# xyzy/jubatus

Measured on AMD Instinct MI355X. Metric: train_samples_per_sec, higher is better.
Workload: dtype fp32

## Files before the change

jubatus_amd/csrc/hip/jb_vc_state.hpp:

```cpp
#pragma once
#include <stdint.h>

#include "jb_serial_layout.hpp"

namespace jb {
namespace vc {

enum : int { kNew = 0, kRetry = 1, kDone = 2, kDense = 3 };
enum : int {
  S_MAGIC = 0, S_BEG, S_BEND, S_STATUS, S_LW, S_T, S_NCAND, S_PEND, S_WHY, S_NUPD, S_NSLOTS, S_VIOL,
  S_DONEB, S_NVALID, S_RETRYW, S_WEND,
  S_WINDOWS, S_RETRIES, S_STEPS, S_ROUNDS, S_WASTED, S_REFRESH, S_EXACT, S_CAND, S_UPD, S_SAT, S_TICKS,
  S_NONC, S_PH0, S_PH1, S_PH2, S_PH3, S_PH4, S_PHW, S_WIDE, S_DENSE_PM,
  S_DCHUNK,
  S_STEPPED,
  S_NCHUNK,
  S_BBEG,
  S_CSMODE,
  S_CSN,
  S_NWORDS = 64
};
enum : int { kWhyEnd = 0, kWhySat = 1, kWhyDense = 2 };
constexpr int64_t kDenseChunk0 = 8192, kDenseChunkMax = 1 << 20;

constexpr int kSpSlotBytes = 98304;
__host__ __device__ constexpr int sp_nslot(int lc) {
  return kSpSlotBytes / (8 * lc) > 1024 ? 1024 : kSpSlotBytes / (8 * lc);
}
__device__ __forceinline__ void sp_buckets(int row, int nb, int* b1, int* b2) {
  const uint32_t h1 = (uint32_t)row * 0x9E3779B1u;
  uint32_t h2 = ((uint32_t)row ^ 0x5bd1e995u) * 0x85EBCA77u;
  h2 ^= h2 >> 13;
  h2 *= 0xC2B2AE35u;
  *b1 = (int)__umulhi(h1, (uint32_t)nb);
  int c = (int)__umulhi(h2, (uint32_t)nb);
  if (c == *b1) c = c + 1 == nb ? 0 : c + 1;
  *b2 = c;
}
__device__ __forceinline__ int sp_find(const int32_t* key, int nb, int32_t row) {
  if (row < 0) return -1;
  int b1, b2;
  sp_buckets(row, nb, &b1, &b2);
  const int4 k1 = reinterpret_cast<const int4*>(key)[b1];
  const int4 k2 = reinterpret_cast<const int4*>(key)[b2];
  int s = -1;
  s = k1.x == row ? 4 * b1 : s;
  s = k1.y == row ? 4 * b1 + 1 : s;
  s = k1.z == row ? 4 * b1 + 2 : s;
  s = k1.w == row ? 4 * b1 + 3 : s;
  s = k2.x == row ? 4 * b2 : s;
  s = k2.y == row ? 4 * b2 + 1 : s;
  s = k2.z == row ? 4 * b2 + 2 : s;
  s = k2.w == row ? 4 * b2 + 3 : s;
  return s;
}

__device__ inline int64_t seg_estimate(const int64_t* st) {
  const int64_t wins = st[S_WINDOWS], stepped = st[S_STEPPED];
  const int64_t committed = st[S_BEG] - st[S_BBEG] - stepped;
  int64_t per = committed > 0 && wins > 0 ? committed / wins : 2048;
  per = per < 1024 ? 1024 : per;
  return wins + st[S_RETRIES] + (stepped + per - 1) / per;
}

}
}
```

jubatus_amd/csrc/hip/serial.hip:

```cpp
#include "jb_linear.hpp"
#include "jb_serial_layout.hpp"
#include <cstdio>
#include <cstdlib>
#include <algorithm>
#include <mutex>
#include <unordered_map>

namespace jb {

constexpr int kCommitThreads = 512;
constexpr int kDBits = 14;
constexpr int kDCap = 1 << kDBits;
constexpr int kDProbe = 32;
constexpr int kDFull = kDCap * 5 / 8;
constexpr int kBloomBits = 16;
constexpr int kSerialNF = 16;
constexpr float kSlackGuard = 1e-4f;
constexpr int kStepBits = 8;
constexpr int kStepCap = 1 << kStepBits;
constexpr int kStepList = 64;
constexpr int kSerialSegments = 4;
constexpr int kSerialSegmentsBig = 48;
constexpr int64_t kSerialBigBatch = 16384;
constexpr int kVerifiedSegmentsMin = 8;
constexpr int kVerifiedSegmentsMax = 2048;
constexpr int kRescoreWaste = 16;
constexpr int kScoreMaxBlocks = 8192;
#ifndef JB_SERIAL_TIMING
#define JB_SERIAL_TIMING 0
#endif
constexpr bool kSerialTiming = JB_SERIAL_TIMING != 0;
__device__ __forceinline__ uint64_t stamp() { return kSerialTiming ? clock64() : 0; }

template <int LC>
__device__ __forceinline__ void sample_scores_ro(const int32_t* __restrict__ fidx,
                                                 const float* __restrict__ fval, int64_t beg, int n,
                                                 const float* __restrict__ W, int lane,
                                                 float (&acc)[Lanes<LC>::K]) {
  using L = Lanes<LC>;
  const int g = lane / L::LW;
  const int l0 = lane % L::LW;
#pragma unroll
  for (int k = 0; k < L::K; ++k) acc[k] = 0.f;
  for (int j = g; j < n; j += L::G) {
    const int32_t idx = fidx[beg + j];
    const float x = fval[beg + j];
    if (idx >= 0) {
      const float* wr = W + (int64_t)idx * LC + l0;
#pragma unroll
      for (int k = 0; k < L::K; ++k) acc[k] += x * wr[64 * k];
    }
  }
#pragma unroll
  for (int off = L::LW; off < 64; off <<= 1) {
#pragma unroll
    for (int k = 0; k < L::K; ++k) acc[k] += __shfl_xor(acc[k], off, 64);
  }
}

template <int LC>
__device__ __forceinline__ float margin_of(const float (&acc)[Lanes<LC>::K], int y,
                                           const bool (&act)[Lanes<LC>::K], int lane, int* lstar,
                                           float* sy_out, float* best_out) {
  using L = Lanes<LC>;
  const int l0 = lane % L::LW;
  float sy = 0.f, best = -INFINITY;
  int bl = -1;
#pragma unroll
  for (int k = 0; k < L::K; ++k) {
    const int l = l0 + 64 * k;
    if (l == y) sy = acc[k];
    if (act[k] && l != y && acc[k] > best) { best = acc[k]; bl = l; }
  }
  sy = __shfl(sy, y % L::LW, 64);
  argmax_wrong<L::LW>(best, bl);
  *lstar = bl;
  *sy_out = sy;
  *best_out = bl >= 0 ? best : 0.f;
  return sy - (bl >= 0 ? best : 0.f);
}

__device__ __forceinline__ float decision_slack(int method, float margin, float nrm, bool has_l,
                                                float C, float sy, float best) {
  float s;
  switch (method) {
    case PERCEPTRON: s = margin; break;
    case PA: case PA1: case PA2:
      if (!(nrm > 0.f)) return INFINITY;
      s = margin - 1.f;
      break;
    case CW: {
      if (!(nrm > 0.f)) return INFINITY;
      s = margin - C * (has_l ? 2.f : 1.f) * nrm;
      break;
    }
    default:
      s = margin - 1.f;
      break;
  }
  const float guard = kSlackGuard * (1.f + fabsf(sy) + fabsf(best));
  if (method == PERCEPTRON ? !(s > guard) : !(s >= guard)) return -1.f;
  return s - guard;
}

template <int LC>
__global__ __launch_bounds__(256) void serial_score_kernel(
    const int64_t* __restrict__ row_ptr, const int32_t* __restrict__ fidx,
    const float* __restrict__ fval, const int32_t* __restrict__ labels,
// ... 470 lines not shown
      if (tid == k) {
        if (!loaded) load_features<NF>(fi, fx, live, nf, fb, fidx, fval);
        s_n = nf;
        s_y = yl;
        s_fb = fb;
        if (nf <= NF)
          for (int u = 0; u < nf; ++u) { s_fi[u] = fi[u]; s_fx[u] = fx[u]; }
      }
      if (wv == 0) {
        d.step_clear(lane);
        __builtin_amdgcn_wave_barrier();
        if (lane == 0) s_sn = 0;
      }
      lds_barrier();
      { const uint64_t t = stamp(); ph[2] += t - tc; tc = t; }
      if (wv == 0) {
        asm volatile("s_waitcnt vmcnt(0)" ::: "memory");
        const int n = s_n;
        bool up;
        if (kStaged && n <= NF)
          up = commit_staged<(LC <= 32 ? LC : 32)>(s_fi, s_fx, n, s_y, W, P, act[0], lane, method, C,
                                                   touched, d);
        else
          up = commit_sample<LC>(fidx, fval, s_fb, n, s_y, W, P, act, lane, method, C, touched, d);
        if (up) ++n_upd; else ++n_waste;
        if (lane == 0) s_waste = n_waste;
      }
      lim = k;
      ++steps;
      ++n_steps;
      { const uint64_t t = stamp(); ph[3] += t - tc; tc = t; }
      lds_barrier();
      { const uint64_t t = stamp(); ph[4] += t - tc; tc = t; }
      tw = stamp();
      if (s_sat || steps > bail_after || (rescore_waste > 0 && s_waste > rescore_waste)) {
        stop = p + k + 1;
        why = s_sat ? kStopSaturated : steps > bail_after ? kStopDense : kStopRescore;
        break;
      }
      if (loaded && open && tid > k && sl >= 0.f) {
        if (s_sn > kStepList || nf > NF) {
          bnd = full_bound();
        } else {
          bnd += d.step_bound<NF>(fi, fx);
        }
      }
    }
    ++n_rounds;
    const bool counted = live && !(sl != sl) && j < stop;
    const uint64_t cm = __builtin_amdgcn_ballot_w64(counted);
    if (lane == 0 && cm != 0) atomicAdd(&s_valid, (unsigned)__popcll(cm));
    if (stop != end) break;
  }
  __syncthreads();
  auto put = [&](int i, int64_t v) { tail[i] = seg == 0 ? v : tail[i] + v; };
  if (lane == 0) put(kTailBoundWave0 + wv, (int64_t)wwork);
  if (tid == 0) {
    tail[kTailStart] = stop;
    tail[kTailEnd] = end;
    tail[kTailReason] = why;
    put(kTailSteps, n_steps);
    put(kTailRounds, n_rounds);
    put(kTailSegments, 1);
    for (int i = 0; i < 6; ++i) put(kTailBoundPhase0 + i, (int64_t)ph[i]);
    put(kTailBoundWall, kSerialTiming ? (int64_t)(wall_clock64() - w0) : 0);
    put(kTailBoundCycles,
        (int64_t)(stamp() - tc) + (int64_t)(ph[0] + ph[1] + ph[2] + ph[3] + ph[4] + ph[5]));
    if (stats != nullptr && s_valid > 0) atomicAdd(stats + 1, (unsigned long long)s_valid);
  }
  if (tid == 0 && stats != nullptr && n_upd > 0) atomicAdd(stats, (unsigned long long)n_upd);
}

}

extern "C" int64_t jb_serial_scratch_bytes(int64_t n_max) {
  return jb::VcScratch::bytes(n_max > 0 ? n_max : 1);
}

extern "C" int64_t jb_serial_scratch_bytes_lc(int64_t n_max, int LC) {
  return LC > 64 ? jb::BoundScratch::bytes(n_max > 0 ? n_max : 1) : jb_serial_scratch_bytes(n_max);
}

enum : int { kSeenReason = 0, kSeenSegments, kSeenSegEst, kSeenWords };
static_assert(jb::kTailSegments == jb::kTailReason + 1, "one copy reads back both");
static std::mutex& seen_mu() {
  static std::mutex mu;
  return mu;
}
static std::unordered_map<void*, int64_t*>& seen_map() {
  static std::unordered_map<void*, int64_t*> seen;
  return seen;
}
static int64_t* segments_seen(void* scratch) {
  std::lock_guard<std::mutex> g(seen_mu());
  auto& seen = seen_map();
  auto it = seen.find(scratch);
  if (it != seen.end()) return it->second;
  int64_t* p = nullptr;
  if (hipHostMalloc((void**)&p, kSeenWords * sizeof(int64_t), hipHostMallocDefault) != hipSuccess) return nullptr;
  p[kSeenReason] = jb::kStopDone;
  p[kSeenSegments] = 128;
  p[kSeenSegEst] = 0;
  seen[scratch] = p;
  return p;
}

extern "C" int jb_vcommit_prepare(const int64_t* row_ptr, const int32_t* fidx, const float* fval,
                                  const int32_t* labels, const int64_t* stream_ptr, int nstreams, int64_t n_max,
                                  float* W, float* S, const int32_t* active, int LC, int method, float C,
                                  unsigned long long* stats, uint8_t* touched, void* scratch, int nseg,
                                  hipStream_t stream);

extern "C" int jb_serial_scratch_forget(void* scratch) {
  std::lock_guard<std::mutex> g(seen_mu());
  auto& seen = seen_map();
  auto it = seen.find(scratch);
  if (it == seen.end()) return 0;
  (void)hipHostFree(it->second);
  seen.erase(it);
  return 1;
}

static int segment_budget(int64_t n_max, int64_t prev, int64_t est, int64_t why) {
  if (n_max < jb::kSerialBigBatch) return jb::kVerifiedSegmentsMin;
  if (why != jb::kStopDone && why != jb::kStopDense) return jb::kVerifiedSegmentsMax;
  static const std::pair<int, int> slack = [] {
    const char* e = getenv("JB_VC_SEG_SLACK");
    int d = 2, c = 8;
    if (e != nullptr && sscanf(e, "%d,%d", &d, &c) != 2) { d = 2; c = 8; }
    return std::make_pair(d > 0 ? d : 2, c >= 0 ? c : 8);
  }();
  prev = std::max(prev, est);
  return (int)std::min<int64_t>(jb::kVerifiedSegmentsMax,
                                std::max<int64_t>(jb::kVerifiedSegmentsMin,
                                                  prev + prev / slack.first + slack.second));
}

extern "C" int jb_serial_prepare(const int64_t* row_ptr, const int32_t* fidx, const float* fval,
                                 const int32_t* labels, const int64_t* stream_ptr, int nstreams,
                                 int64_t n_max, float* W, float* S, const int32_t* active, int LC,
                                 int method, float C, unsigned long long* stats, uint8_t* touched,
                                 void* scratch, int64_t scratch_bytes, int bail_after,
                                 hipStream_t stream) {
  if (nstreams <= 0 || n_max <= 0) return 0;
  if (scratch == nullptr || scratch_bytes < jb_serial_scratch_bytes_lc(n_max, LC)) return -3;
  if (method >= jb::CW && S == nullptr) return -4;
  int64_t* tail = (int64_t*)scratch;
  if (LC <= 64) {
    volatile int64_t* seen = segments_seen(scratch);
    const int nseg = seen != nullptr
                         ? segment_budget(n_max, seen[kSeenSegments], seen[kSeenSegEst], seen[kSeenReason])
                         : segment_budget(n_max, 0, 0, jb::kStopDone);
    const int rc = jb_vcommit_prepare(row_ptr, fidx, fval, labels, stream_ptr, nstreams, n_max, W, S, active,
                                      LC, method, C, stats, touched, scratch, nseg, stream);
    if (rc == 0 && seen != nullptr) {
      int64_t* host = const_cast<int64_t*>(seen);
      (void)hipMemcpyAsync(host + kSeenReason, tail + jb::kTailReason, 2 * sizeof(int64_t), hipMemcpyDeviceToHost,
                           stream);
      (void)hipMemcpyAsync(host + kSeenSegEst, tail + jb::kTailSegEst, sizeof(int64_t), hipMemcpyDeviceToHost,
                           stream);
    }
    return rc;
  }
  float* slack = (float*)((uint8_t*)scratch + jb::BoundScratch::slack_offset());
  float* l1n = (float*)((uint8_t*)scratch + jb::BoundScratch::l1_offset(n_max));
  const int64_t blocks = std::min<int64_t>((n_max * 64 + 255) / 256, jb::kScoreMaxBlocks);
  const int nseg = n_max >= jb::kSerialBigBatch ? jb::kSerialSegmentsBig : jb::kSerialSegments;
  static_assert(jb::kTailStart == 0 && jb::kTailEnd == 1, "the tail doubles as a one-stream stream_ptr");
  for (int seg = 0; seg < nseg; ++seg) {
    const int waste = seg + 1 < nseg ? jb::kRescoreWaste : 0;
    const int64_t* sp = seg == 0 ? stream_ptr : tail;
    const int ns = seg == 0 ? nstreams : 1;
    const int64_t* why = seg == 0 ? nullptr : tail + jb::kTailReason;
#define JB_SERIAL(L)                                                                              \
  hipLaunchKernelGGL((jb::serial_score_kernel<L>), dim3((unsigned)blocks), dim3(256), 0, stream,  \
                     row_ptr, fidx, fval, labels, sp, ns, W, active, method, C, slack, l1n, why); \
  hipLaunchKernelGGL((jb::serial_commit_kernel<L>), dim3(1), dim3(jb::kCommitThreads), 0, stream, \
                     row_ptr, fidx, fval, labels, sp, ns, W, S, active, method, C, slack, l1n,    \
                     stats, touched, tail, bail_after, seg, waste);                               \
  break;
    switch (LC) {
      case 128: JB_SERIAL(128)
      case 256: JB_SERIAL(256)
      case 512: JB_SERIAL(512)
      case 1024: JB_SERIAL(1024)
      default: return -1;
    }
#undef JB_SERIAL
  }
  return (int)hipGetLastError();
}
```

jubatus_amd/csrc/hip/vcommit.hip:

```cpp
#include <string.h>

#include <type_traits>

#include "jb_commit.hpp"
#include "jb_vc_state.hpp"

namespace jb {
namespace vc {

using dc::Geo;
constexpr int kFCMax = 2;
constexpr int kRec = 16 * kFCMax;
constexpr int64_t kLwMin = 2048, kLwMax = kVcWindowMax, kLwInit = 8192;
constexpr int kBitWords = kVcBitWords;
constexpr float kTInit = 0.5f, kTMin = 0.125f, kTMax = 64.f;
constexpr int64_t kMagic = 0x56434f4d4d495433LL;
constexpr int kRetryForce = 3;

__device__ __forceinline__ float st_T(const int64_t* st) { return __int_as_float((int)st[S_T]); }
__device__ __forceinline__ int64_t ld_st(const int64_t* p) {
  return __hip_atomic_load(p, __ATOMIC_RELAXED, __HIP_MEMORY_SCOPE_AGENT);
}
__device__ __forceinline__ bool live(int status) { return status == kNew || status == kRetry; }

__device__ __forceinline__ float frcp(float x) { return __builtin_amdgcn_rcpf(x); }
__device__ __forceinline__ bool step_coeffs_fast(int method, float margin, float var, float nrm, bool has_l, float C,
                                                 float* tau, float* beta) {
  switch (method) {
    case PERCEPTRON:
      if (margin <= 0.f) { *tau = 1.f; *beta = 0.f; return true; }
      return false;
    case PA: case PA1: case PA2: {
      const float loss = 1.f - margin;
      if (!(loss > 0.f && nrm > 0.f)) return false;
      const float sq = (has_l ? 2.f : 1.f) * nrm;
      if (method == PA) *tau = loss * frcp(sq);
      else if (method == PA1) *tau = fminf(C, loss * frcp(sq));
      else *tau = loss * frcp(sq + 0.5f * frcp(C));
      *beta = 0.f;
      return true;
    }
    case CW: {
      if (!(var > 0.f)) return false;
      const float phi = C;
      const float b = 1.f + 2.f * phi * margin;
      const float disc = b * b - 8.f * phi * (margin - phi * var);
      const float gamma = (-b + sqrtf(fmaxf(disc, 0.f))) * frcp(4.f * phi * var);
      if (!(gamma > 0.f)) return false;
      *tau = gamma; *beta = 2.f * gamma * phi;
      return true;
    }
    case AROW:
      if (!(margin < 1.f)) return false;
      *beta = frcp(var + frcp(C));
      *tau = (1.f - margin) * *beta;
      return true;
    case NHERD: {
      if (!(margin < 1.f)) return false;
      *tau = (1.f - margin) * frcp(var + frcp(C));
      const float cv = 1.f + C * var;
      *beta = (C * C * var + 2.f * C) * frcp(cv * cv);
      return true;
    }
    default: return false;
  }
}
__device__ __forceinline__ float dprec_fast(int method, float beta, float x, float s) {
  const float bx2 = beta * x * x;
  return method == CW ? bx2 : bx2 * frcp(1.f - bx2 * s);
}

__global__ __launch_bounds__(256) void vc_init_kernel(int64_t* __restrict__ st, const int64_t* __restrict__ sp,
                                                      int nstreams, unsigned long long* __restrict__ bits,
                                                      int64_t* __restrict__ tail, float t_force,
                                                      int32_t* __restrict__ g_key, float* __restrict__ g_rmax,
                                                      int dense_pm) {
  for (int i = threadIdx.x; i < kBitWords; i += blockDim.x) bits[i] = 0ull;
  const bool fresh = st[S_MAGIC] != kMagic;
  if (fresh)
    for (int i = threadIdx.x; i < 1024; i += blockDim.x) { g_key[i] = -1; g_rmax[i] = 0.f; }
  __syncthreads();
  if (threadIdx.x != 0) return;
  if (fresh) {
    for (int i = 0; i < S_NWORDS; ++i) st[i] = 0;
    st[S_MAGIC] = kMagic;
    st[S_LW] = kLwInit;
    st[S_T] = __float_as_int(kTInit);
  }
  if (t_force > 0.f) st[S_T] = __float_as_int(t_force);
  const int64_t beg = sp[0], bend = sp[nstreams];
  st[S_BEG] = beg;
  st[S_BEND] = bend;
  st[S_WEND] = beg;
  st[S_STATUS] = beg < bend ? kNew : kDone;
  for (int i = S_NCAND; i <= S_RETRYW; ++i) st[i] = 0;
  for (int i = S_WINDOWS; i < S_NWORDS; ++i) st[i] = 0;
// ... 139 lines not shown
    const int64_t pn = st[S_NCAND], pu = st[S_NUPD];
    st[S_CSMODE] = (cs_min > 0 && ncand >= cs_min && pu * 1000 >= (int64_t)cs_pm * (pn > 0 ? pn : 1)) ? 1 : 0;
    st[S_NCAND] = ncand;
    st[S_WEND] = we;
  }
  const int64_t nwaves = (int64_t)gridDim.x * (blockDim.x >> 6);
  const int g = lane / L::LW;
  const int l0 = lane % L::LW;
  const bool la = l0 < LC && active[l0] != 0;
  for (int64_t k = ((int64_t)blockIdx.x * blockDim.x + tid) >> 6; k < ncand; k += nwaves) {
    int lo = 0, hi = nw - 1;
    while (lo < hi) {
      const int mid = (lo + hi + 1) >> 1;
      if (s_pref[mid] <= k) lo = mid; else hi = mid - 1;
    }
    unsigned long long word = bits[lo];
    for (int j = (int)k - s_pref[lo]; j > 0; --j) word &= word - 1;
    const int pos = 64 * lo + (__ffsll((long long)word) - 1);
    const int64_t s = beg + pos;
    int n;
    float acc, q;
    wave_score<LC>(row_ptr, fidx, fval, W, s, lane, la, &n, &acc, &q);
    const int64_t fb = row_ptr[s];
    if (lane < kRec) {
      const bool in = lane < n;
      FI[k * kRec + lane] = in ? fidx[fb + lane] : -1;
      FX[k * kRec + lane] = in ? fval[fb + lane] : 0.f;
    }
    if (lane == 0 && n > 16) atomicOr((unsigned long long*)&st[S_WIDE], 1ull);
    if (lane < LC) S0[k * LC + lane] = acc;
    (void)g;
    const int y = labels[s];
    if (y < 0 || y >= LC) {
      if (lane == 0) AUX[k] = make_int4(dc::aux_pack(-1, -1, n), __float_as_int(q), __float_as_int(1.f), pos);
      continue;
    }
    int bl;
    const float sl0 = wave_slack<LC>(acc, y, la, lane, method, C, q, &bl);
    if (lane == 0) AUX[k] = make_int4(dc::aux_pack(y, bl, n), __float_as_int(q), __float_as_int(sl0), pos);
    if (P == nullptr) continue;
    if (lane < kRec) {
      float2 pp = make_float2(1.f, 1.f);
      if (lane < n) {
        const int32_t idx = fidx[fb + lane];
        if (idx >= 0) {
          pp.x = P[(int64_t)idx * LC + y];
          if (bl >= 0) pp.y = P[(int64_t)idx * LC + bl];
        }
      }
      PP0[k * kRec + lane] = pp;
    }
  }
}

template <int LC, int FC>
struct Raw {
  int32_t fi[FC];
  float fx[FC];
  float2 pp[FC];
  float s[Geo<LC>::K];
  int aux;
  float nrm;
  float slack0;
  int pos;
};

template <int LC, int FC>
struct Samp {
  int32_t fi[FC];
  float fx[FC];
  float py[FC];
  float pl[FC];
  float s[Geo<LC>::K];
  int y;
  int ls0;
  int nf;
  float nrm;
  float slack0;
  int pos;
};

struct __attribute__((aligned(16))) Stamp { float sid, dy, dl, rmax; };

template <int LC, int MT, int R_, int PD_, int FC_>
__global__ __launch_bounds__(64) void vc_commit_kernel(
    int64_t* __restrict__ st, const float* __restrict__ W, const float* __restrict__ P,
    const int32_t* __restrict__ active, float C, const float* __restrict__ S0_k,
    const int4* __restrict__ AUX_k, const float2* __restrict__ PP0_k, const int32_t* __restrict__ FI_k,
    const float* __restrict__ FX_k, int32_t* __restrict__ g_key, float* __restrict__ g_rmax,
    float* __restrict__ g_dw, float* __restrict__ g_dp, int prof) {
  using Gm = Geo<LC>;
  using Rw = Raw<LC, FC_>;
  using S = Samp<LC, FC_>;
  constexpr int kFC = FC_;
  constexpr int kNFM = 16 * FC_;
  constexpr int kR = R_;
  constexpr int kNS = 4 * R_;
  constexpr int kPD = PD_;
  constexpr int K = Gm::K;
  constexpr int NSLOT = Gm::NSLOT;
  constexpr int method = MT;
  constexpr bool use_s = MT >= CW;
  constexpr bool use_nrm = MT == PA || MT == PA1 || MT == PA2 || MT == CW;
  constexpr float kG = dc::kGuard;
  if (!live((int)st[S_STATUS])) return;
  if (st[S_CSMODE] == 1) return;
  if ((st[S_WIDE] != 0) != (FC_ == 2)) return;
  __shared__ __attribute__((aligned(16))) float s_dw[NSLOT * LC + Gm::PAD];
  __shared__ __attribute__((aligned(16))) float s_dp[use_s ? NSLOT * LC + Gm::PAD : 4];
  __shared__ __attribute__((aligned(16))) int32_t s_key[NSLOT];
  __shared__ __attribute__((aligned(16))) Stamp s_sg[NSLOT + 1];

  const int lane = threadIdx.x;
  const int sub = lane & 15;
  const int G = lane >> 4;
  const uint64_t t_k0 = __builtin_amdgcn_s_memrealtime();
  const uint64_t t_c0 = __builtin_amdgcn_s_memtime();
  {
    float4* dw4 = reinterpret_cast<float4*>(s_dw);
    float4* dp4 = reinterpret_cast<float4*>(s_dp);
    const float4 z = make_float4(0.f, 0.f, 0.f, 0.f);
    for (int i = lane; i < (NSLOT * LC + Gm::PAD) / 4; i += 64) {
      dw4[i] = z;
      if (use_s) dp4[i] = z;
    }
    for (int i = lane; i < NSLOT; i += 64) s_key[i] = -1;
    for (int i = lane; i <= NSLOT; i += 64) s_sg[i] = Stamp{__int_as_float(-1), 0.f, 0.f, 0.f};
  }
  int act[K];
#pragma unroll
  for (int k = 0; k < K; ++k) {
    const int lab = sub + 16 * k;
    act[k] = (lab < LC && active[lab] != 0) ? 1 : 0;
  }
  const int64_t ncand = (int64_t)dc::in_vgpr((uint64_t)st[S_NCAND]);
  const int64_t wb = (int64_t)dc::in_vgpr((uint64_t)st[S_BEG]);
  const int64_t we = (int64_t)dc::in_vgpr((uint64_t)st[S_WEND]);
  const float* __restrict__ S0 = dc::in_vgpr(S0_k);
  const int4* __restrict__ AUX = dc::in_vgpr(AUX_k);
  const float2* __restrict__ PP0 = dc::in_vgpr(PP0_k);
  const int32_t* __restrict__ FI = dc::in_vgpr(FI_k);
  const float* __restrict__ FX = dc::in_vgpr(FX_k);

  auto load_raw = [&](int64_t k0, Rw (&rw)[kR]) {
#pragma unroll
    for (int r = 0; r < kR; ++r) {
      int64_t j = k0 + G * kR + r;
      j = j < ncand ? j : ncand - 1;
      j = j < 0 ? 0 : j;
#pragma unroll
      for (int c = 0; c < kFC; ++c) {
        const int64_t o = j * kRec + c * 16 + sub;
        rw[r].fi[c] = dc::gld(FI + o);
        rw[r].fx[c] = dc::gld(FX + o);
        if (use_s) rw[r].pp[c] = dc::gld(PP0 + o);
      }
#pragma unroll
      for (int k = 0; k < K; ++k) {
        const int lab = sub + 16 * k;
        rw[r].s[k] = dc::gld(S0 + j * LC + (lab < LC ? lab : LC - 1));
      }
      const int* a = reinterpret_cast<const int*>(AUX + j);
      rw[r].aux = dc::gld(a);
      rw[r].slack0 = __int_as_float(dc::gld(a + 2));
      rw[r].pos = dc::gld(a + 3);
      if (use_nrm) rw[r].nrm = __int_as_float(dc::gld(a + 1));
    }
  };
  auto unpack = [&](int64_t k0, const Rw (&rw)[kR], S (&sm)[kR]) {
#pragma unroll
    for (int r = 0; r < kR; ++r) {
      const bool ok = k0 + G * kR + r < ncand;
#pragma unroll
      for (int c = 0; c < kFC; ++c) {
        sm[r].fi[c] = ok ? rw[r].fi[c] : -1;
        sm[r].fx[c] = ok ? rw[r].fx[c] : 0.f;
        sm[r].py[c] = (use_s && ok) ? rw[r].pp[c].x : 1.f;
        sm[r].pl[c] = (use_s && ok) ? rw[r].pp[c].y : 1.f;
      }
#pragma unroll
      for (int k = 0; k < K; ++k) sm[r].s[k] = (ok && sub + 16 * k < LC) ? rw[r].s[k] : 0.f;
      const int aux = rw[r].aux;
      sm[r].y = ok ? dc::aux_y(aux) : -1;
      sm[r].ls0 = (use_s && ok) ? dc::aux_ls(aux) : -1;
      sm[r].nf = ok ? dc::aux_nf(aux) : 0;
      sm[r].nrm = (use_nrm && ok) ? rw[r].nrm : 0.f;
      sm[r].slack0 = ok ? rw[r].slack0 : 1.f;
      sm[r].pos = rw[r].pos;
    }
  };

  S sc[kR];
  Rw pf[kPD][kR];
#pragma unroll
  for (int i = 0; i < kPD; ++i) load_raw((int64_t)i * kNS, pf[i]);

  int stopped = 0;
  int64_t pend = we;
  int why = kWhyEnd;
  int n_steps = 0, n_exact = 0;
  __shared__ int s_cnt[4];
  __shared__ unsigned long long s_ph[5];
  if (lane < 4) s_cnt[lane] = 0;
  if (lane < 5) s_ph[lane] = 0;
  auto bump = [&](int i) __attribute__((always_inline)) {
    if (lane == 0) s_cnt[i] += 1;
  };
  const uint64_t kLead = 0x0001000100010001ull;

  const bool kProf = prof != 0;

  uint64_t tp = kProf ? __builtin_amdgcn_s_memtime() : 0;
  auto stamp = [&](int i) __attribute__((always_inline)) {
    if (!kProf) return;
    const uint64_t t = __builtin_amdgcn_s_memtime();
    if (lane == 0) s_ph[i] += t - tp;
    tp = t;
  };
  auto round = [&](int64_t k0) __attribute__((always_inline)) {
    int alive[kR], unsafe[kR], exact[kR];
    float slack[kR];
    int slot[kR][kFC];
    bool widew = false;
#pragma unroll
    for (int r = 0; r < kR; ++r) {
      alive[r] = (sc[r].y >= 0 && sc[r].y < LC) ? 1 : 0;
      widew |= alive[r] && sc[r].nf > 16;
    }
    const bool two = kFC == 2 && __builtin_amdgcn_ballot_w64(widew) != 0;
#pragma unroll
    for (int r = 0; r < kR; ++r) {
      const bool ok = alive[r] && sc[r].nf <= kNFM;
      slot[r][0] = ok ? dc::cache_find<LC>(s_key, sc[r].fi[0]) : -1;
      if (kFC == 2) slot[r][kFC - 1] = (two && ok) ? dc::cache_find<LC>(s_key, sc[r].fi[kFC - 1]) : -1;
    }
    auto make_exact = [&](int after) {
      bool need[kR];
      bool anyneed = false;
#pragma unroll
      for (int r = 0; r < kR; ++r) {
        need[r] = alive[r] && !exact[r] && sc[r].nf <= kNFM && G * kR + r > after && !(slack[r] > 0.f);
        anyneed |= need[r];
      }
      if (__builtin_amdgcn_ballot_w64(anyneed) == 0) return;
#pragma unroll
      for (int r = 0; r < kR; ++r) {
        if (__builtin_amdgcn_ballot_w64(need[r]) == 0) continue;
        float t[K];
#pragma unroll
        for (int k = 0; k < K; ++k) t[k] = sc[r].s[k];
        dc::row_correct<LC, kFC>(s_dw, slot[r], sc[r].fx, sub, two, t);
        int ls;
        float sy, best;
        const float m = dc::group_margin<LC>(t, sc[r].y, act, sub, &ls, &sy, &best);
        const float sl = dc::slack_of(method, m, sc[r].nrm, ls >= 0, C, sy, best);
        if (need[r]) {
#pragma unroll
          for (int k = 0; k < K; ++k) sc[r].s[k] = t[k];
          slack[r] = sl;
          exact[r] = 1;
          if (sub == 0) ++n_exact;
        }
      }
    };
#pragma unroll
    for (int r = 0; r < kR; ++r) {
      float bsum = 0.f;
#pragma unroll
      for (int c = 0; c < kFC; ++c)
        bsum += slot[r][c] >= 0 ? fabsf(sc[r].fx[c]) * s_sg[slot[r][c]].rmax : 0.f;
      slack[r] = sc[r].slack0 - 2.f * (1.f + 4.f * kG) * row16_sum(bsum);
      exact[r] = 0;
    }
    make_exact(-1);
    stamp(0);
#pragma unroll
    for (int r = 0; r < kR; ++r) unsafe[r] = (alive[r] && (sc[r].nf > kNFM || !(slack[r] > 0.f))) ? 1 : 0;

    int lim = -1;
    for (;;) {
      int k = dc::kInf;
#pragma unroll
      for (int r = 0; r < kR; ++r) {
        const uint64_t b = __builtin_amdgcn_ballot_w64(unsafe[r] && G * kR + r > lim) & kLead;
        if (b != 0) {
// ... 175 lines not shown
            cy = row16_sum(cy);
            cl = row16_sum(cl);
            if (exact[r]) {
#pragma unroll
              for (int kk = 0; kk < K; ++kk) {
                const int lab = sub + 16 * kk;
                if (lab == yk) sc[r].s[kk] += cy;
                if (lab == lk) sc[r].s[kk] += cl;
              }
            }
            slack[r] -= (fabsf(cy) + fabsf(cl)) * (1.f + 4.f * kG);
            if (exact[r] && !(slack[r] > 0.f)) {
              int ls2;
              float sy2, best2;
              const float m2 = dc::group_margin<LC>(sc[r].s, sc[r].y, act, sub, &ls2, &sy2, &best2);
              slack[r] = dc::slack_of(method, m2, sc[r].nrm, ls2 >= 0, C, sy2, best2);
            }
          }
          make_exact(k);
#pragma unroll
          for (int r = 0; r < kR; ++r)
            if (G * kR + r > k) unsafe[r] = (alive[r] && (sc[r].nf > kNFM || !(slack[r] > 0.f))) ? 1 : 0;
        }
        return 0;
      };
      int stop_code = 0;
      switch (rk) {
        case 0: stop_code = step_of(std::integral_constant<int, 0>{}); break;
        case 1: if constexpr (kR > 1) stop_code = step_of(std::integral_constant<int, (kR > 1 ? 1 : 0)>{}); break;
        case 2: if constexpr (kR > 2) stop_code = step_of(std::integral_constant<int, (kR > 2 ? 2 : 0)>{}); break;
        default: if constexpr (kR > 3) stop_code = step_of(std::integral_constant<int, (kR > 3 ? 3 : 0)>{}); break;
      }
      stamp(4);
      if (stop_code) break;
      lim = k;
    }
    bump(3);
  };
  for (int64_t p0 = 0; p0 < ncand && !stopped; p0 += kPD * kNS) {
#pragma unroll
    for (int u = 0; u < kPD; ++u) {
      const int64_t p = p0 + u * kNS;
      unpack(p, pf[u], sc);
      load_raw(p + kPD * kNS, pf[u]);
      if (p < ncand && !stopped) round(p);
    }
  }
  int nslots = 0;
  for (int i = lane; i < NSLOT; i += 64) {
    const int32_t key = s_key[i];
    g_key[i] = key;
    g_rmax[i] = s_sg[i].rmax;
    nslots += key >= 0;
  }
  {
    constexpr int Q = LC / 4;
    for (int i = lane; i < NSLOT * Q; i += 64) {
      if (s_key[i / Q] < 0) continue;
      reinterpret_cast<float4*>(g_dw)[i] = reinterpret_cast<const float4*>(s_dw)[i];
      if (use_s) reinterpret_cast<float4*>(g_dp)[i] = reinterpret_cast<const float4*>(s_dp)[i];
    }
  }
#pragma unroll
  for (int off = 1; off < 64; off <<= 1) nslots += __shfl_xor(nslots, off, 64);
  if (lane == 0) {
    st[S_PEND] = pend;
    st[S_WHY] = why;
    st[S_NUPD] = s_cnt[0];
    st[S_NSLOTS] = nslots;
    st[S_STEPS] += n_steps;
    st[S_ROUNDS] += s_cnt[3];
    st[S_WASTED] += s_cnt[1];
    st[S_REFRESH] += s_cnt[2];
    st[S_EXACT] += n_exact;
    st[S_CAND] += ncand;
    st[S_TICKS] += (int64_t)(__builtin_amdgcn_s_memrealtime() - t_k0);
    if (kProf) {
      for (int i = 0; i < 5; ++i) st[S_PH0 + i] += (int64_t)s_ph[i];
      st[S_PHW] += (int64_t)(__builtin_amdgcn_s_memtime() - t_c0);
    }
  }
}

template <int LC>
__global__ __launch_bounds__(256) void vc_verify_kernel(
    int64_t* __restrict__ st, const int64_t* __restrict__ row_ptr, const int32_t* __restrict__ fidx,
    const float* __restrict__ fval, const int32_t* __restrict__ labels, const float* __restrict__ SL,
    unsigned long long* __restrict__ bits, const int32_t* __restrict__ g_key,
    const float* __restrict__ g_rmax, const float* __restrict__ g_dw, const float* __restrict__ g_dp,
    float* __restrict__ W, float* __restrict__ P, uint8_t* __restrict__ touched,
    unsigned long long* __restrict__ stats, int64_t* __restrict__ tail) {
  using Gm = Geo<LC>;
  constexpr int NSLOT = Gm::NSLOT;
  constexpr float kG = dc::kGuard;
  const int status = (int)st[S_STATUS];
  if (!live(status)) return;
  __shared__ __attribute__((aligned(16))) int32_t s_key[NSLOT];
  __shared__ float s_rmax[NSLOT];
  __shared__ unsigned s_valid, s_viol;
  __shared__ int s_last, s_force;
  const int tid = threadIdx.x;
  for (int i = tid; i < NSLOT; i += blockDim.x) {
    s_key[i] = g_key[i];
    s_rmax[i] = g_rmax[i];
  }
  if (tid == 0) { s_valid = 0; s_viol = 0; }
  __syncthreads();
  const int64_t wb = st[S_BEG], pe = st[S_PEND];
  const bool cs_mode = st[S_CSMODE] == 1;
  unsigned nvalid = 0, nviol = 0, nnonc = 0;
  for (int64_t i = wb + (int64_t)blockIdx.x * blockDim.x + tid; i < pe; i += (int64_t)gridDim.x * blockDim.x) {
    const int y = labels[i];
    if (y < 0 || y >= LC) continue;
    ++nvalid;
    const int64_t rel = i - wb;
    const unsigned long long bit = 1ull << (rel & 63);
    if (bits[rel >> 6] & bit) continue;
    ++nnonc;
    float bound = 0.f;
    for (int64_t j = row_ptr[i]; j < row_ptr[i + 1]; ++j) {
      const int32_t row = fidx[j];
      if (row < 0) continue;
      const int s = cs_mode ? sp_find(s_key, sp_nslot(LC) / 4, row) : dc::cache_find<LC>(s_key, row);
      if (s >= 0) bound += fabsf(fval[j]) * s_rmax[s];
    }
    bound *= 2.f * (1.f + 4.f * kG);
    if (!(SL[rel] > bound)) {
      atomicOr(bits + (rel >> 6), bit);
      ++nviol;
    }
  }
  if (nvalid) atomicAdd(&s_valid, nvalid);
  if (nviol) atomicAdd(&s_viol, nviol);
  if (nnonc) atomicAdd((unsigned long long*)&st[S_NONC], (unsigned long long)nnonc);
  __syncthreads();
  if (tid == 0) {
    if (s_valid) atomicAdd((unsigned long long*)&st[S_NVALID], (unsigned long long)s_valid);
    if (s_viol) atomicAdd((unsigned long long*)&st[S_VIOL], (unsigned long long)s_viol);
    __threadfence();
    s_last = atomicAdd((unsigned long long*)&st[S_DONEB], 1ull) == (unsigned long long)(gridDim.x - 1);
  }
  __syncthreads();
  if (!s_last) return;
  __threadfence();
  const int64_t viol = ld_st(&st[S_VIOL]);
  const int64_t wend = st[S_WEND];
  if (viol == 0) {
    __shared__ int s_used[NSLOT];
    __shared__ int s_nused;
    if (tid == 0) s_nused = 0;
    __syncthreads();
    for (int i = tid; i < NSLOT; i += blockDim.x)
      if (s_key[i] >= 0) s_used[atomicAdd(&s_nused, 1)] = i;
    __syncthreads();
    constexpr int Q = LC / 4;
    constexpr int kU = 4;
    const int items = s_nused * Q;
    for (int b0 = 0; b0 < items; b0 += kU * (int)blockDim.x) {
      float4 w[kU], d[kU], pv[kU], dp[kU];
      int64_t off[kU];
      bool on[kU];
#pragma unroll
      for (int u = 0; u < kU; ++u) {
        const int it = b0 + u * (int)blockDim.x + tid;
        on[u] = it < items;
        const int sl = s_used[on[u] ? it / Q : 0];
        const int q = it % Q;
        off[u] = (int64_t)s_key[sl] * Q + q;
        const int gi = sl * Q + q;
        if (on[u]) {
          w[u] = reinterpret_cast<const float4*>(W)[off[u]];
          d[u] = reinterpret_cast<const float4*>(g_dw)[gi];
          if (P != nullptr) {
            pv[u] = reinterpret_cast<const float4*>(P)[off[u]];
            dp[u] = reinterpret_cast<const float4*>(g_dp)[gi];
          }
        }
      }
#pragma unroll
      for (int u = 0; u < kU; ++u) {
        if (!on[u]) continue;
        w[u].x += d[u].x; w[u].y += d[u].y; w[u].z += d[u].z; w[u].w += d[u].w;
        reinterpret_cast<float4*>(W)[off[u]] = w[u];
        if (P != nullptr) {
          pv[u].x += dp[u].x; pv[u].y += dp[u].y; pv[u].z += dp[u].z; pv[u].w += dp[u].w;
          reinterpret_cast<float4*>(P)[off[u]] = pv[u];
        }
        if (off[u] % Q == 0 && touched != nullptr) touched[off[u] / Q] = 1;
      }
    }
    for (int i = tid; i < kBitWords; i += blockDim.x) bits[i] = 0ull;
    if (tid == 0) {
      const int64_t nupd = st[S_NUPD];
      const int64_t nv = ld_st(&st[S_NVALID]);
      if (stats != nullptr) {
        if (nupd > 0) atomicAdd(stats, (unsigned long long)nupd);
        if (nv > 0) atomicAdd(stats + 1, (unsigned long long)nv);
      }
      const int why = (int)st[S_WHY];
      const int64_t bend = st[S_BEND];
      st[S_BEG] = pe;
      st[S_WINDOWS] += 1;
      st[S_UPD] += nupd;
      if (why == kWhySat) st[S_SAT] += 1;
      const int64_t dpm = st[S_DENSE_PM];
      const bool dense = dpm > 0 && pe < bend && nupd * 1000 > dpm * (pe - wb);
      st[S_STATUS] = (why == kWhyDense || dense) ? kDense : (pe >= bend ? kDone : kNew);
      if (!(why == kWhyDense || dense)) st[S_DCHUNK] = kDenseChunk0;
      int64_t lw = st[S_LW];
      if (why == kWhySat) {
        const int64_t took = pe - wb;
        lw = took + took / 4;
      } else if (pe - wb >= lw) {
        lw = 2 * lw;
      }
      lw = lw < kLwMin ? kLwMin : (lw > kLwMax ? kLwMax : lw);
      st[S_LW] = lw;
      const float T = fmaxf(kTMin, st_T(st) * 0.97f);
      st[S_T] = __float_as_int(T);
      st[S_RETRYW] = 0;
    }
  } else {
    if (tid == 0) {
      st[S_RETRIES] += 1;
      st[S_RETRYW] += 1;
      const float T = fminf(kTMax, st_T(st) * 1.5f);
      st[S_T] = __float_as_int(T);
// ... 1 lines not shown
      s_force = st[S_RETRYW] >= kRetryForce;
    }
    __syncthreads();
    if (s_force) {
      const int64_t n = wend - wb;
      for (int64_t w = tid; w < (n + 63) / 64; w += blockDim.x) {
        const int64_t rem = n - 64 * w;
        bits[w] = rem >= 64 ? ~0ull : ((1ull << rem) - 1);
      }
    }
  }
  __syncthreads();
  if (tid == 0) {
    st[S_DONEB] = 0;
    st[S_NVALID] = 0;
    st[S_VIOL] = 0;
    const int s2 = (int)st[S_STATUS];
    if (s2 != kRetry) st[S_WIDE] = 0;
    tail[kTailStart] = s2 == kDone ? st[S_BEND] : st[S_BEG];
    tail[kTailEnd] = st[S_BEND];
    tail[kTailSteps] = st[S_STEPS];
    tail[kTailRounds] = st[S_ROUNDS];
    tail[kTailReason] = s2 == kDone ? kStopDone : s2 == kDense ? kStopDense : kStopSaturated;
    tail[kTailSegments] = st[S_WINDOWS] + st[S_RETRIES];
    tail[kTailStepped] = st[S_STEPPED];
    tail[kTailChunks] = st[S_NCHUNK];
    tail[kTailSegEst] = seg_estimate(st);
    tail[kTailCsWindows] = st[S_CSN];
    tail[kTailWasted] = st[S_WASTED];
    tail[kTailRefresh] = st[S_REFRESH];
    tail[kTailUpdates] = st[S_UPD];
    tail[kTailRows] = st[S_NSLOTS];
    tail[kTailExact] = st[S_EXACT];
    tail[kTailCand] = st[S_CAND];
    tail[kTailRetries] = st[S_RETRIES];
    tail[kTailSatWindows] = st[S_SAT];
    tail[kTailTicks] = st[S_TICKS];
    for (int i = 0; i < 5; ++i) tail[kTailVcPhase0 + i] = st[S_PH0 + i];
    tail[kTailVcPhaseWall] = st[S_PHW];
    tail[kTailVcWindowLen] = st[S_LW];
    tail[kTailVcT] = st[S_T];
    tail[kTailVcNonCand] = st[S_NONC];
  }
}

}
}

extern "C" int64_t jb_vcommit_fixed_bytes() { return jb::kVcFixed; }

extern "C" int jb_stepper_enabled();
extern "C" int jb_stepper_chunk(const int64_t* row_ptr, const int32_t* fidx, const float* fval, const int32_t* labels,
                                float* W, float* P, const int32_t* active, int LC, int method, float C,
                                unsigned long long* stats, uint8_t* touched, int64_t* vst, int64_t* vtail,
                                hipStream_t stream);
extern "C" int jb_stepper_cand(const int64_t* row_ptr, const int32_t* fidx, const float* fval,
                               const int32_t* labels, float* W, float* P, const int32_t* active, int LC, int method,
                               float C, int64_t* vst, const int4* aux, int32_t* g_key, float* g_rmax, float* g_dw,
                               float* g_dp, hipStream_t stream);

template <int L>
static int launch_vc(int method, const int64_t* row_ptr, const int32_t* fidx, const float* fval,
                     const int32_t* labels, float* W, float* S, const int32_t* active, float C, int64_t* st,
                     float* sl, unsigned long long* bits, float* s0, int4* aux, float2* pp0, int32_t* fi,
                     float* fx, int32_t* gk, float* gr, float* gdw, float* gdp, uint8_t* touched,
                     unsigned long long* stats, int64_t* tail, int nseg, bool chunks, int cs_min, int cs_pm,
                     hipStream_t stream) {
  using namespace jb::vc;
  static const int prof = [] {
    const char* e = getenv("JB_COMMIT_PROF");
    return (e != nullptr && e[0] == '1') ? 1 : 0;
  }();
  static const bool r1pd1 = [] {
    const char* e = getenv("JB_VC_SHAPE");
    return e != nullptr && strcmp(e, "r1pd1") == 0;
  }();
  float* Pp = method >= jb::CW ? S : nullptr;
  for (int seg = 0; seg < nseg; ++seg) {
    hipLaunchKernelGGL((vc_score_kernel<L>), dim3(1024), dim3(256), 0, stream, st, row_ptr, fidx, fval, labels,
                       W, active, method, C, sl, bits, gk, gr);
    hipLaunchKernelGGL((vc_gather_kernel<L>), dim3(512), dim3(256), 0, stream, st, row_ptr, fidx, fval, labels,
                       W, Pp, active, method, C, bits, s0, aux, pp0, fi, fx, cs_min, cs_pm);
#define JB_VC_S(M, R, PD)                                                                                       \
  hipLaunchKernelGGL((vc_commit_kernel<L, M, R, PD, 1>), dim3(1), dim3(64), 0, stream, st, W, Pp, active, C, s0, \
                     aux, pp0, fi, fx, gk, gr, gdw, gdp, prof);                                                  \
  hipLaunchKernelGGL((vc_commit_kernel<L, M, R, PD, 2>), dim3(1), dim3(64), 0, stream, st, W, Pp, active, C, s0, \
                     aux, pp0, fi, fx, gk, gr, gdw, gdp, prof);
#define JB_VC_M(M)                               \
  if (r1pd1) { JB_VC_S(M, 1, 1) }                \
  else { JB_VC_S(M, 1, 2) }                      \
  break;
    switch (method) {
      case jb::PERCEPTRON: JB_VC_M(jb::PERCEPTRON)
      case jb::PA: JB_VC_M(jb::PA)
      case jb::PA1: JB_VC_M(jb::PA1)
      case jb::PA2: JB_VC_M(jb::PA2)
      case jb::CW: JB_VC_M(jb::CW)
      case jb::AROW: JB_VC_M(jb::AROW)
      case jb::NHERD: JB_VC_M(jb::NHERD)
      default: return -1;
    }
#undef JB_VC_M
#undef JB_VC_S
    if (cs_min > 0) {
      const int rc = jb_stepper_cand(row_ptr, fidx, fval, labels, W, Pp, active, L, method, C, st, aux, gk, gr, gdw,
                                     gdp, stream);
      if (rc != 0) return rc;
    }
    hipLaunchKernelGGL((vc_verify_kernel<L>), dim3(256), dim3(256), 0, stream, st, row_ptr, fidx, fval, labels,
                       sl, bits, gk, gr, gdw, gdp, W, Pp, touched, stats, tail);
    if (chunks) {
      const int rc = jb_stepper_chunk(row_ptr, fidx, fval, labels, W, Pp, active, L, method, C, stats, touched, st,
                                      tail, stream);
      if (rc != 0) return rc;
    }
  }
  return 0;
}

extern "C" int jb_vcommit_prepare(const int64_t* row_ptr, const int32_t* fidx, const float* fval,
                                  const int32_t* labels, const int64_t* stream_ptr, int nstreams, int64_t n_max,
                                  float* W, float* S, const int32_t* active, int LC, int method, float C,
                                  unsigned long long* stats, uint8_t* touched, void* scratch, int nseg,
                                  hipStream_t stream) {
  if (LC > 64) return -1;
  using Lay = jb::VcScratch;
  int64_t* tail = (int64_t*)scratch;
  uint8_t* base = (uint8_t*)scratch;
  float* s0 = (float*)(base + Lay::offset(Lay::S0, n_max));
  float2* pp0 = (float2*)(base + Lay::offset(Lay::PP0, n_max));
  int32_t* fi = (int32_t*)(base + Lay::offset(Lay::FI, n_max));
  float* fx = (float*)(base + Lay::offset(Lay::FX, n_max));
  int4* aux = (int4*)(base + Lay::offset(Lay::AUX, n_max));
  float* sl = (float*)(base + Lay::offset(Lay::SL, n_max));
  uint8_t* fixed = base + Lay::fixed_offset(n_max);
  int64_t* st = (int64_t*)fixed;
  unsigned long long* bits = (unsigned long long*)(fixed + jb::kVcStateBytes);
  int32_t* gk = (int32_t*)(bits + jb::kVcBitWords);
  float* gr = (float*)(gk + jb::kVcStoreRows);
  float* gdw = gr + jb::kVcStoreRows;
  float* gdp = gdw + jb::kVcStoreFloats;
  const char* te = getenv("JB_VERIFIED_T");
  const float t_force = te != nullptr ? (float)atof(te) : 0.f;
  const char* de = getenv("JB_VC_DENSE_PM");
  const int dense_pm = de != nullptr ? atoi(de) : 300;
  hipLaunchKernelGGL(jb::vc::vc_init_kernel, dim3(1), dim3(256), 0, stream, st, stream_ptr, nstreams, bits, tail,
                     t_force, gk, gr, dense_pm);
  const bool chunks = dense_pm > 0 && jb_stepper_enabled();
  const char* cs_e = getenv("JB_VC_CS");
  const char* cs_p = getenv("JB_VC_CS_PM");
  const int cs_min = (jb_stepper_enabled() && cs_e != nullptr) ? atoi(cs_e) : 0;
  const int cs_pm = cs_p != nullptr ? atoi(cs_p) : 350;
  int rc = 0;
#define JB_VC_L(L)                                                                                            \
  rc = launch_vc<L>(method, row_ptr, fidx, fval, labels, W, S, active, C, st, sl, bits, s0, aux, pp0, fi, fx, \
                    gk, gr, gdw, gdp, touched, stats, tail, nseg, chunks, cs_min, cs_pm, stream);              \
  break;
  switch (LC) {
    case 8: JB_VC_L(8)
    case 16: JB_VC_L(16)
    case 32: JB_VC_L(32)
    case 64: JB_VC_L(64)
    default: return -1;
  }
#undef JB_VC_L
  if (rc) return rc;
  return (int)hipGetLastError();
}
```

Before: 269.9 million.

## Merge commit kernel variants, parallelize verify per row, retune segment budget

Folds the two FC-specialized single-block commit launches into one kernel that picks the wide or narrow body at runtime, removing one launch per segment. The verify kernel now uses 16 lanes per sample with a row16 reduction instead of one thread per sample, and only stages the slot cache in blocks that have work. The host segment budget starts at a fixed first-call value, uses different slack defaults and a stronger estimate-based growth term, retries count double in the estimate, and the minimum window shrinks. The risks are a larger combined kernel with more register or LDS pressure, and budgets that over- or under-provision segments.

```diff
diff --git a/jubatus_amd/csrc/hip/jb_vc_state.hpp b/jubatus_amd/csrc/hip/jb_vc_state.hpp
--- a/jubatus_amd/csrc/hip/jb_vc_state.hpp
+++ b/jubatus_amd/csrc/hip/jb_vc_state.hpp
@@ -60,7 +60,7 @@
   const int64_t committed = st[S_BEG] - st[S_BBEG] - stepped;
   int64_t per = committed > 0 && wins > 0 ? committed / wins : 2048;
   per = per < 1024 ? 1024 : per;
-  return wins + st[S_RETRIES] + (stepped + per - 1) / per;
+  return wins + 2 * st[S_RETRIES] + (stepped + per - 1) / per;
 }
 
 }
diff --git a/jubatus_amd/csrc/hip/serial.hip b/jubatus_amd/csrc/hip/serial.hip
--- a/jubatus_amd/csrc/hip/serial.hip
+++ b/jubatus_amd/csrc/hip/serial.hip
@@ -24,6 +24,7 @@
 constexpr int64_t kSerialBigBatch = 16384;
 constexpr int kVerifiedSegmentsMin = 8;
 constexpr int kVerifiedSegmentsMax = 2048;
+constexpr int kVerifiedSegmentsFirst = 200;
 constexpr int kRescoreWaste = 16;
 constexpr int kScoreMaxBlocks = 8192;
 #ifndef JB_SERIAL_TIMING
@@ -660,6 +661,7 @@
 }
 
 enum : int { kSeenReason = 0, kSeenSegments, kSeenSegEst, kSeenWords };
+constexpr int64_t kSeenFresh = -1;
 static_assert(jb::kTailSegments == jb::kTailReason + 1, "one copy reads back both");
 static std::mutex& seen_mu() {
   static std::mutex mu;
@@ -676,8 +678,8 @@
   if (it != seen.end()) return it->second;
   int64_t* p = nullptr;
   if (hipHostMalloc((void**)&p, kSeenWords * sizeof(int64_t), hipHostMallocDefault) != hipSuccess) return nullptr;
-  p[kSeenReason] = jb::kStopDone;
-  p[kSeenSegments] = 128;
+  p[kSeenReason] = kSeenFresh;
+  p[kSeenSegments] = 0;
   p[kSeenSegEst] = 0;
   seen[scratch] = p;
   return p;
@@ -701,17 +703,17 @@
 
 static int segment_budget(int64_t n_max, int64_t prev, int64_t est, int64_t why) {
   if (n_max < jb::kSerialBigBatch) return jb::kVerifiedSegmentsMin;
+  if (why == kSeenFresh) return jb::kVerifiedSegmentsFirst;
   if (why != jb::kStopDone && why != jb::kStopDense) return jb::kVerifiedSegmentsMax;
   static const std::pair<int, int> slack = [] {
     const char* e = getenv("JB_VC_SEG_SLACK");
-    int d = 2, c = 8;
-    if (e != nullptr && sscanf(e, "%d,%d", &d, &c) != 2) { d = 2; c = 8; }
-    return std::make_pair(d > 0 ? d : 2, c >= 0 ? c : 8);
+    int d = 8, c = 4;
+    if (e != nullptr && sscanf(e, "%d,%d", &d, &c) != 2) { d = 8; c = 4; }
+    return std::make_pair(d > 0 ? d : 8, c >= 0 ? c : 4);
   }();
-  prev = std::max(prev, est);
-  return (int)std::min<int64_t>(jb::kVerifiedSegmentsMax,
-                                std::max<int64_t>(jb::kVerifiedSegmentsMin,
-                                                  prev + prev / slack.first + slack.second));
+  int64_t want = prev + prev / slack.first + slack.second;
+  if (est > prev) want = std::max(want, est + est / 2 + 8);
+  return (int)std::min<int64_t>(jb::kVerifiedSegmentsMax, std::max<int64_t>(jb::kVerifiedSegmentsMin, want));
 }
 
 extern "C" int jb_serial_prepare(const int64_t* row_ptr, const int32_t* fidx, const float* fval,
diff --git a/jubatus_amd/csrc/hip/vcommit.hip b/jubatus_amd/csrc/hip/vcommit.hip
--- a/jubatus_amd/csrc/hip/vcommit.hip
+++ b/jubatus_amd/csrc/hip/vcommit.hip
@@ -11,7 +11,7 @@
 using dc::Geo;
 constexpr int kFCMax = 2;
 constexpr int kRec = 16 * kFCMax;
-constexpr int64_t kLwMin = 2048, kLwMax = kVcWindowMax, kLwInit = 8192;
+constexpr int64_t kLwMin = 256, kLwMax = kVcWindowMax, kLwInit = 8192;
 constexpr int kBitWords = kVcBitWords;
 constexpr float kTInit = 0.5f, kTMin = 0.125f, kTMax = 64.f;
 constexpr int64_t kMagic = 0x56434f4d4d495433LL;
@@ -317,13 +317,22 @@
 
 struct __attribute__((aligned(16))) Stamp { float sid, dy, dl, rmax; };
 
+struct CommitLds {
+  float* dw;
+  float* dp;
+  int32_t* key;
+  Stamp* sg;
+  int* cnt;
+  unsigned long long* ph;
+};
+
 template <int LC, int MT, int R_, int PD_, int FC_>
-__global__ __launch_bounds__(64) void vc_commit_kernel(
+__device__ __forceinline__ void vc_commit_body(
     int64_t* __restrict__ st, const float* __restrict__ W, const float* __restrict__ P,
     const int32_t* __restrict__ active, float C, const float* __restrict__ S0_k,
     const int4* __restrict__ AUX_k, const float2* __restrict__ PP0_k, const int32_t* __restrict__ FI_k,
     const float* __restrict__ FX_k, int32_t* __restrict__ g_key, float* __restrict__ g_rmax,
-    float* __restrict__ g_dw, float* __restrict__ g_dp, int prof) {
+    float* __restrict__ g_dw, float* __restrict__ g_dp, int prof, const CommitLds lds) {
   using Gm = Geo<LC>;
   using Rw = Raw<LC, FC_>;
   using S = Samp<LC, FC_>;
@@ -338,13 +347,12 @@
   constexpr bool use_s = MT >= CW;
   constexpr bool use_nrm = MT == PA || MT == PA1 || MT == PA2 || MT == CW;
   constexpr float kG = dc::kGuard;
-  if (!live((int)st[S_STATUS])) return;
-  if (st[S_CSMODE] == 1) return;
-  if ((st[S_WIDE] != 0) != (FC_ == 2)) return;
-  __shared__ __attribute__((aligned(16))) float s_dw[NSLOT * LC + Gm::PAD];
-  __shared__ __attribute__((aligned(16))) float s_dp[use_s ? NSLOT * LC + Gm::PAD : 4];
-  __shared__ __attribute__((aligned(16))) int32_t s_key[NSLOT];
-  __shared__ __attribute__((aligned(16))) Stamp s_sg[NSLOT + 1];
+  float* const s_dw = lds.dw;
+  float* const s_dp = lds.dp;
+  int32_t* const s_key = lds.key;
+  Stamp* const s_sg = lds.sg;
+  int* const s_cnt = lds.cnt;
+  unsigned long long* const s_ph = lds.ph;
 
   const int lane = threadIdx.x;
   const int sub = lane & 15;
@@ -434,8 +442,6 @@
   int64_t pend = we;
   int why = kWhyEnd;
   int n_steps = 0, n_exact = 0;
-  __shared__ int s_cnt[4];
-  __shared__ unsigned long long s_ph[5];
   if (lane < 4) s_cnt[lane] = 0;
   if (lane < 5) s_ph[lane] = 0;
   auto bump = [&](int i) __attribute__((always_inline)) {
@@ -777,6 +783,33 @@
   }
 }
 
+template <int LC, int MT, int R_, int PD_>
+__global__ __launch_bounds__(64) void vc_commit_kernel(
+    int64_t* __restrict__ st, const float* __restrict__ W, const float* __restrict__ P,
+    const int32_t* __restrict__ active, float C, const float* __restrict__ S0_k,
+    const int4* __restrict__ AUX_k, const float2* __restrict__ PP0_k, const int32_t* __restrict__ FI_k,
+    const float* __restrict__ FX_k, int32_t* __restrict__ g_key, float* __restrict__ g_rmax,
+    float* __restrict__ g_dw, float* __restrict__ g_dp, int prof) {
+  using Gm = Geo<LC>;
+  constexpr int NSLOT = Gm::NSLOT;
+  constexpr bool use_s = MT >= CW;
+  if (!live((int)st[S_STATUS])) return;
+  if (st[S_CSMODE] == 1) return;
+  __shared__ __attribute__((aligned(16))) float s_dw[NSLOT * LC + Gm::PAD];
+  __shared__ __attribute__((aligned(16))) float s_dp[use_s ? NSLOT * LC + Gm::PAD : 4];
+  __shared__ __attribute__((aligned(16))) int32_t s_key[NSLOT];
+  __shared__ __attribute__((aligned(16))) Stamp s_sg[NSLOT + 1];
+  __shared__ int s_cnt[4];
+  __shared__ unsigned long long s_ph[5];
+  const CommitLds lds{s_dw, s_dp, s_key, s_sg, s_cnt, s_ph};
+  if (st[S_WIDE] != 0)
+    vc_commit_body<LC, MT, R_, PD_, 2>(st, W, P, active, C, S0_k, AUX_k, PP0_k, FI_k, FX_k, g_key, g_rmax, g_dw,
+                                       g_dp, prof, lds);
+  else
+    vc_commit_body<LC, MT, R_, PD_, 1>(st, W, P, active, C, S0_k, AUX_k, PP0_k, FI_k, FX_k, g_key, g_rmax, g_dw,
+                                       g_dp, prof, lds);
+}
+
 template <int LC>
 __global__ __launch_bounds__(256) void vc_verify_kernel(
     int64_t* __restrict__ st, const int64_t* __restrict__ row_ptr, const int32_t* __restrict__ fidx,
@@ -795,32 +828,47 @@
   __shared__ unsigned s_valid, s_viol;
   __shared__ int s_last, s_force;
   const int tid = threadIdx.x;
-  for (int i = tid; i < NSLOT; i += blockDim.x) {
-    s_key[i] = g_key[i];
-    s_rmax[i] = g_rmax[i];
-  }
+  const int sub = tid & 15;
+  const int64_t wb = st[S_BEG], pe = st[S_PEND];
+  const bool cs_mode = st[S_CSMODE] == 1;
+  const int64_t row0 = ((int64_t)blockIdx.x * blockDim.x) >> 4;
+  const int64_t nrows = ((int64_t)gridDim.x * blockDim.x) >> 4;
+  const bool has = wb + row0 < pe;
+  auto stage = [&]() {
+    for (int i = tid; i < NSLOT; i += blockDim.x) {
+      s_key[i] = g_key[i];
+      s_rmax[i] = g_rmax[i];
+    }
+  };
+  if (has) stage();
   if (tid == 0) { s_valid = 0; s_viol = 0; }
   __syncthreads();
-  const int64_t wb = st[S_BEG], pe = st[S_PEND];
-  const bool cs_mode = st[S_CSMODE] == 1;
   unsigned nvalid = 0, nviol = 0, nnonc = 0;
-  for (int64_t i = wb + (int64_t)blockIdx.x * blockDim.x + tid; i < pe; i += (int64_t)gridDim.x * blockDim.x) {
+  for (int64_t i = wb + row0 + (tid >> 4); i < pe; i += nrows) {
     const int y = labels[i];
-    if (y < 0 || y >= LC) continue;
-    ++nvalid;
     const int64_t rel = i - wb;
     const unsigned long long bit = 1ull << (rel & 63);
-    if (bits[rel >> 6] & bit) continue;
-    ++nnonc;
-    float bound = 0.f;
-    for (int64_t j = row_ptr[i]; j < row_ptr[i + 1]; ++j) {
-      const int32_t row = fidx[j];
-      if (row < 0) continue;
-      const int s = cs_mode ? sp_find(s_key, sp_nslot(LC) / 4, row) : dc::cache_find<LC>(s_key, row);
-      if (s >= 0) bound += fabsf(fval[j]) * s_rmax[s];
-    }
-    bound *= 2.f * (1.f + 4.f * kG);
-    if (!(SL[rel] > bound)) {
+    const unsigned long long word = bits[rel >> 6];
+    const int64_t fb = row_ptr[i];
+    const int n = (int)(row_ptr[i + 1] - fb);
+    const float sl0 = SL[rel];
+    if (y < 0 || y >= LC) continue;
+    if (sub == 0) ++nvalid;
+    if (word & bit) continue;
+    if (sub == 0) ++nnonc;
+    float b = 0.f;
+    for (int j0 = 0; j0 < n; j0 += 16) {
+      const bool in = j0 + sub < n;
+      const int64_t j = fb + (in ? j0 + sub : j0);
+      const int32_t r = fidx[j];
+      const float x = fval[j];
+      const int32_t row = in ? r : -1;
+      const int sl = cs_mode ? sp_find(s_key, sp_nslot(LC) / 4, row) : dc::cache_find<LC>(s_key, row);
+      const float rm = s_rmax[sl >= 0 ? sl : 0];
+      b += sl >= 0 ? fabsf(x) * rm : 0.f;
+    }
+    const float bound = row16_sum(b) * (2.f * (1.f + 4.f * kG));
+    if (sub == 0 && !(sl0 > bound)) {
       atomicOr(bits + (rel >> 6), bit);
       ++nviol;
     }
@@ -838,6 +886,10 @@
   __syncthreads();
   if (!s_last) return;
   __threadfence();
+  if (!has) {
+    stage();
+    __syncthreads();
+  }
   const int64_t viol = ld_st(&st[S_VIOL]);
   const int64_t wend = st[S_WEND];
   if (viol == 0) {
@@ -1005,9 +1057,7 @@
     hipLaunchKernelGGL((vc_gather_kernel<L>), dim3(512), dim3(256), 0, stream, st, row_ptr, fidx, fval, labels,
                        W, Pp, active, method, C, bits, s0, aux, pp0, fi, fx, cs_min, cs_pm);
 #define JB_VC_S(M, R, PD)                                                                                       \
-  hipLaunchKernelGGL((vc_commit_kernel<L, M, R, PD, 1>), dim3(1), dim3(64), 0, stream, st, W, Pp, active, C, s0, \
-                     aux, pp0, fi, fx, gk, gr, gdw, gdp, prof);                                                  \
-  hipLaunchKernelGGL((vc_commit_kernel<L, M, R, PD, 2>), dim3(1), dim3(64), 0, stream, st, W, Pp, active, C, s0, \
+  hipLaunchKernelGGL((vc_commit_kernel<L, M, R, PD>), dim3(1), dim3(64), 0, stream, st, W, Pp, active, C, s0, \
                      aux, pp0, fi, fx, gk, gr, gdw, gdp, prof);
 #define JB_VC_M(M)                               \
   if (r1pd1) { JB_VC_S(M, 1, 1) }                \
```

Result: slower. 262.0 million (-2.9%).
